# wengflow/robust-e-nerf

Measured on AMD Instinct MI355X. Metric: train_rays_per_sec, higher is better.
Workload: dtype f32; 1 GPU; BASELINE configs[1]: synthetic ficus-like event stream, 65536 events/step/GPU = 2 renders x 65536 rays x 128 samples, arch ngp, fp32, l_diff (2 renders), fwd+bwd+Adam; sampler=uniform; sampler=uniform, samples_per_ray=128, parallelism=dp1, front_prefetched=False, mlp_precision=highest, device_counts=False, device_count_overflows=0, fwd_chunks=8, dist_world_size=1

## Files before the change

robust_e_nerf_amd/csrc/ren_hashgrid_binned.hip:

```cpp
#include <cstdlib>
#include "ren_hashgrid_common.h"

namespace {

constexpr int BIN_SHIFT = 13;
constexpr int BIN_ENTRIES = 1 << BIN_SHIFT;
constexpr int MAX_BINS_PER_LEVEL = 64;
constexpr int MAX_BINS = REN_MAX_LEVELS * MAX_BINS_PER_LEVEL;
#ifndef REN_SC_THREADS
#define REN_SC_THREADS 512
#endif
#ifndef REN_SC_WAVES
#define REN_SC_WAVES 6
#endif
#ifndef REN_SC_WAVES_PAIR
#define REN_SC_WAVES_PAIR 8
#endif
constexpr int SC_THREADS = REN_SC_THREADS;
constexpr int SC_ENTRIES = SC_THREADS * 8;
constexpr int CNT_THREADS = 1024, CNT_SAMPLES = 1024;
constexpr int64_t PART_ENTRIES_MIN = 1 << 16, PART_ENTRIES_MAX = 1 << 23;
constexpr int N_SUB = 8;
__device__ __forceinline__ int xcd_id() {
    unsigned x;
    asm volatile("s_getreg_b32 %0, hwreg(HW_REG_XCC_ID)" : "=s"(x));
    return (int)(x & (N_SUB - 1));
}
inline int64_t part_entries_for(int64_t n, int64_t hashed_cap) {
    int64_t p = hashed_cap;
    if (p == 0) {
        p = PART_ENTRIES_MIN;
        while (p < (1 << 21) && p * 1024 < n * 128) p <<= 1;
    }
    return p < PART_ENTRIES_MIN ? PART_ENTRIES_MIN : (p > PART_ENTRIES_MAX ? PART_ENTRIES_MAX : p);
}
constexpr int LMAX_SLOTS = 8, LMAX_STRIDE = 32;
constexpr int LMAX_WORDS = REN_MAX_LEVELS * LMAX_SLOTS * LMAX_STRIDE;

struct BinTab {
    int bin_base[REN_MAX_LEVELS + 1];
    uint32_t cap[REN_MAX_LEVELS];
    uint32_t pair[REN_MAX_LEVELS];
    uint32_t skip[REN_MAX_LEVELS];
    int sub_by_xcd;
    int cnt_stride;
    int halve;
};

struct Part {
    uint32_t gbin, single;
    uint64_t begin, end;
};

struct Workspace {
    uint32_t *counts, *level_max, *cursors, *n_parts;
    uint32_t *bin_cap;
    uint64_t *bin_start;
    Part *parts;
    char *pool;
};
constexpr int PAIR_BIN_SHIFT = 26;

struct TanSrc {
    const float *rays_do, *rays_dd, *dfeatd;
};

__device__ __forceinline__ void lds_barrier() { asm volatile("s_waitcnt lgkmcnt(0)\n\ts_barrier" ::: "memory"); }

struct SampleArgs {
    int layout;
    const float *dfeat, *x_unit;
    ren_scene_dev sc;
    const float *rays_o, *rays_d;
    const int32_t *ray_indices;
    const float *t_starts, *t_ends;
    int64_t n;
    TanSrc tan;
    const int64_t *n_dev;
};

template <bool TAN>
__device__ __forceinline__ void unit_pos(const SampleArgs &a, int64_t i, float *u, float *ud) {
    ud[0] = 0.f; ud[1] = 0.f; ud[2] = 0.f;
    if (TAN) {
        float x[3], xd[3];
        sample_pos_jvp(a.rays_o, a.rays_d, a.tan.rays_do, a.tan.rays_dd, a.ray_indices, a.t_starts, a.t_ends, i, x, xd);
        contract_jvp(a.sc, x, xd, u, ud);
    } else if (a.x_unit) {
        u[0] = a.x_unit[3 * i]; u[1] = a.x_unit[3 * i + 1]; u[2] = a.x_unit[3 * i + 2];
    } else {
        float x, y, z; int ray;
        ren_sample_pos(a.rays_o, a.rays_d, a.ray_indices, a.t_starts, a.t_ends, i, x, y, z, ray);
        ren_contract(a.sc, x, y, z, u[0], u[1], u[2]);
    }
}

template <bool TAN>
__device__ __forceinline__ bool load_dfeat(const SampleArgs &a, int n_levels, int lvl, int64_t i, float &d0, float &d1,
                                           float &e0, float &e1) {
    e0 = 0.f; e1 = 0.f;
    if (TAN || a.layout == 1) {
        const int64_t b = ((i >> 5) * REN_MAX_LEVELS + lvl) * 64 + (i & 31);
        d0 = a.dfeat[b]; d1 = a.dfeat[b + 32];
        if (TAN) { e0 = a.tan.dfeatd[b]; e1 = a.tan.dfeatd[b + 32]; }
    } else {
        const float2 d = reinterpret_cast<const float2 *>(a.dfeat)[i * n_levels + lvl];
        d0 = d.x; d1 = d.y;
    }
    return d0 != 0.f || d1 != 0.f || e0 != 0.f || e1 != 0.f;
}


constexpr int RUN_LANES = 16;

template <int OFF>
__device__ __forceinline__ float dpp_shr(float v) {
    return __int_as_float(__builtin_amdgcn_update_dpp(0, __float_as_int(v), 0x110 | OFF, 0xf, 0xf, true));
}
template <int OFF>
__device__ __forceinline__ int dpp_shr_i(int v) { return __builtin_amdgcn_update_dpp(0, v, 0x110 | OFF, 0xf, 0xf, true); }

__device__ __forceinline__ bool run_tail(bool dense, bool have, uint32_t key, int lane, bool &head) {
    if (!dense) { head = true; return have; }
    const uint32_t k = have ? key : 0x80000000u | (uint32_t)lane;
    const uint32_t kp = __shfl_up(k, 1, 64), kn = __shfl_down(k, 1, 64);
    const int sub = lane & (RUN_LANES - 1);
    head = !(sub > 0 && have && kp == k);
    return have && (sub == RUN_LANES - 1 || kn != k);
}

template <int OFF>
__device__ __forceinline__ void run_merge_step(int &f, float (&v0)[8], float (&v1)[8]) {
    const float take = f ? 0.f : 1.f;
#pragma unroll
    for (int c = 0; c < 8; ++c) {
        v0[c] = fmaf(dpp_shr<OFF>(v0[c]), take, v0[c]);
        v1[c] = fmaf(dpp_shr<OFF>(v1[c]), take, v1[c]);
    }
    f |= dpp_shr_i<OFF>(f);
}

__device__ __forceinline__ void run_merge(bool head, int lane, float (&v0)[8], float (&v1)[8]) {
    int f = head ? 1 : 0;
    run_merge_step<1>(f, v0, v1);
    run_merge_step<2>(f, v0, v1);
    run_merge_step<4>(f, v0, v1);
    run_merge_step<8>(f, v0, v1);
}

__device__ __forceinline__ uint32_t bin_rank(bool dense, bool emit, uint32_t bin, int lane, uint32_t *hist) {
    if (!dense) return emit ? atomicAdd(&hist[bin], 1u) : 0u;
    uint32_t rank = 0;
    uint64_t todo = __ballot(emit);
    while (todo) {
        const int leader = __ffsll((unsigned long long)todo) - 1;
        const uint32_t b = __shfl(bin, leader, 64);
        const uint64_t m = __ballot(emit && bin == b);
        uint32_t base = 0;
        if (lane == leader) base = atomicAdd(&hist[b], (uint32_t)__popcll(m));
        base = __shfl(base, leader, 64);
        if (emit && bin == b) rank = base + (uint32_t)__popcll(m & ((1ull << lane) - 1ull));
        todo &= ~m;
    }
    return rank;
}

__device__ __forceinline__ void bin_rank8_dense(bool emit, const uint32_t (&bin)[8], int lane, uint32_t *hist, uint32_t (&rank)[8]) {
    const uint64_t m = __ballot(emit);
#pragma unroll
    for (int c = 0; c < 8; ++c) rank[c] = 0;
    if (!m) return;
    const int leader = __ffsll((unsigned long long)m) - 1;
    uint32_t lb[8];
    bool mixed = false;
#pragma unroll
    for (int c = 0; c < 8; ++c) {
        lb[c] = __shfl(bin[c], leader, 64);
        mixed |= emit && bin[c] != lb[c];
    }
    if (__ballot(mixed)) {
#pragma unroll
        for (int c = 0; c < 8; ++c) rank[c] = bin_rank(true, emit, bin[c], lane, hist);
        return;
    }
    const uint32_t cnt = (uint32_t)__popcll(m), pre = (uint32_t)__popcll(m & ((1ull << lane) - 1ull));
    uint32_t base[8] = {0, 0, 0, 0, 0, 0, 0, 0};
    if (lane == leader) {
#pragma unroll
        for (int c = 0; c < 8; ++c) base[c] = atomicAdd(&hist[lb[c]], cnt);
    }
#pragma unroll
    for (int c = 0; c < 8; ++c) rank[c] = __shfl(base[c], leader, 64) + pre;
}

template <bool TAN>
__global__ __launch_bounds__(CNT_THREADS) void bin_count_kernel(GridDev g, BinTab bt, SampleArgs a,
                                                                uint32_t *__restrict__ counts) {
    __shared__ uint32_t hist[MAX_BINS];
    for (int t = threadIdx.x; t < MAX_BINS; t += CNT_THREADS) hist[t] = 0;
    __syncthreads();
    const int lane = threadIdx.x & 63;
#pragma unroll 1
    for (int k = 0; k < CNT_SAMPLES / CNT_THREADS; ++k) {
        const int64_t i = (int64_t)blockIdx.x * bt.cnt_stride * CNT_SAMPLES + k * CNT_THREADS + threadIdx.x;
        const bool inb = i < ren_eff_n(a.n, a.n_dev);
        float u[3] = {0.f, 0.f, 0.f}, ud[3];
        if (inb) unit_pos<TAN>(a, i, u, ud);
#pragma unroll 1
        for (int lvl = 0; lvl < g.n_levels; ++lvl) {
            if (bt.cap[lvl] || bt.skip[lvl]) continue;
            float d0, d1, e0, e1;
            const bool have = inb && (a.dfeat == nullptr || load_dfeat<TAN>(a, g.n_levels, lvl, i, d0, d1, e0, e1));
            const LevelPos p = level_pos(u[0], u[1], u[2], g.scale[lvl]);
            const uint32_t res = g.res[lvl], size = g.size[lvl];
            const bool hashed = g.hashed[lvl] != 0;
            bool head;
            uint32_t idx[8];
            corner_indices8(p.c[0], p.c[1], p.c[2], res, size, hashed, idx);
            const bool emit = run_tail(!hashed, have, idx[0], lane, head);
#pragma unroll
            for (int c = 0; c < 8; ++c) (void)bin_rank(!hashed, emit, idx[c] >> BIN_SHIFT, lane, hist + lvl * MAX_BINS_PER_LEVEL);
        }
    }
    __syncthreads();
    for (int t = threadIdx.x; t < MAX_BINS; t += CNT_THREADS) {
        const int lvl = t / MAX_BINS_PER_LEVEL, bin = t % MAX_BINS_PER_LEVEL;
        if (lvl < g.n_levels && bin < bt.bin_base[lvl + 1] - bt.bin_base[lvl] && hist[t])
            atomicAdd(&counts[bt.bin_base[lvl] + bin], hist[t]);
    }
}

__global__ __launch_bounds__(MAX_BINS) void bin_offsets_kernel(int n_bins, BinTab bt, uint64_t capacity_slots,
                                                               const uint32_t *__restrict__ counts,
                                                               uint32_t *__restrict__ cursors,
                                                               uint32_t *__restrict__ bin_cap,
                                                               uint64_t *__restrict__ bin_start) {
    __shared__ uint64_t s_cnt[MAX_BINS];
    const int t = threadIdx.x;
    uint64_t c = 0, slots = 0;
    bool pair = false;
    if (t < n_bins) {
        int lvl = 0;
        while (lvl + 1 < REN_MAX_LEVELS && t >= bt.bin_base[lvl + 1]) ++lvl;
        pair = bt.pair[lvl] != 0;
        c = bt.skip[lvl] ? 0 : bt.cap[lvl] ? bt.cap[lvl] : counts[t];
        if (!bt.skip[lvl] && !bt.cap[lvl] && bt.cnt_stride > 1) c = c * bt.cnt_stride + c * bt.cnt_stride / 4 + 4096;
        if (bt.halve) c = c / 2;
        c &= ~(uint64_t)7;
        if (pair) c = (c / N_SUB) & ~(uint64_t)7;
        slots = pair ? c * N_SUB : (c * 10 + 15) / 16;
        for (int x = 0; x < N_SUB; ++x) cursors[t * N_SUB + x] = 0;
    }
    s_cnt[t] = slots;
    __syncthreads();
    for (int off = 1; off < MAX_BINS; off <<= 1) {
        const uint64_t a = t >= off ? s_cnt[t - off] : 0;
        __syncthreads();
        s_cnt[t] += a;
        __syncthreads();
    }
    if (t < n_bins) {
        const uint64_t start = s_cnt[t] - slots;
        uint64_t room = start < capacity_slots ? capacity_slots - start : 0;
        if (room > slots) room = slots;
        if (room < slots) c = (pair ? room / N_SUB : room * 16 / 10) & ~(uint64_t)7;
        bin_start[t] = start < capacity_slots ? start : capacity_slots;
        bin_cap[t] = (uint32_t)c;
    }
    if (t == n_bins - 1) bin_start[n_bins] = s_cnt[t] < capacity_slots ? s_cnt[t] : capacity_slots;
}

__global__ __launch_bounds__(MAX_BINS) void bin_partition_kernel(int n_bins, uint64_t PART_ENTRIES, BinTab bt,
                                                                 const uint32_t *__restrict__ cursors,
                                                                 const uint32_t *__restrict__ bin_cap,
                                                                 Part *__restrict__ parts, uint32_t *__restrict__ n_parts) {
    __shared__ uint32_t s_np[MAX_BINS];
    const int t = threadIdx.x;
    uint64_t c = 0;
    bool pair = false;
    if (t < n_bins) {
        int lvl = 0;
        while (lvl + 1 < REN_MAX_LEVELS && t >= bt.bin_base[lvl + 1]) ++lvl;
        pair = bt.pair[lvl] != 0;
        for (int x = 0; x < (pair ? N_SUB : 1); ++x) c += cursors[t * N_SUB + x] < bin_cap[t] ? cursors[t * N_SUB + x] : bin_cap[t];
    }
    const uint32_t np = pair ? (c ? 1u : 0u) : (uint32_t)((c + PART_ENTRIES - 1) / PART_ENTRIES);
    s_np[t] = np;
    __syncthreads();
    for (int off = 1; off < MAX_BINS; off <<= 1) {
        const uint32_t b = t >= off ? s_np[t - off] : 0;
        __syncthreads();
        s_np[t] += b;
        __syncthreads();
    }
    if (t == n_bins - 1) n_parts[0] = s_np[t];
    const uint32_t pbase = s_np[t] - np;
    for (uint32_t k = 0; k < np; ++k) {
        Part p;
        p.gbin = t; p.single = np == 1;
        p.begin = (uint64_t)k * PART_ENTRIES;
        p.end = k + 1 == np ? c : p.begin + PART_ENTRIES;
        parts[pbase + k] = p;
    }
}

__device__ __forceinline__ void table_atomic(float *grad_table, uint32_t offset, uint32_t idx, float a, float b) {
    float *gt = grad_table + 2 * ((size_t)offset + idx);
    atomicAdd(gt, a);
    atomicAdd(gt + 1, b);
}

template <bool TAN, int KIND>
__global__ __launch_bounds__(SC_THREADS, KIND == 1 ? REN_SC_WAVES_PAIR : REN_SC_WAVES) void bin_scatter_kernel(
    GridDev g, BinTab bt, SampleArgs a, Workspace ws, float *__restrict__ grad_table) {
    __shared__ uint32_t hist[MAX_BINS_PER_LEVEL], loc[MAX_BINS_PER_LEVEL + 1], fit[MAX_BINS_PER_LEVEL];
    __shared__ char *gp0[MAX_BINS_PER_LEVEL], *gp1[MAX_BINS_PER_LEVEL];
    __shared__ __attribute__((aligned(16))) unsigned char stage[KIND == 1 ? SC_THREADS * 4 * 16 : SC_ENTRIES * 12];
    __shared__ float wave_max[SC_THREADS / 64];
    __shared__ int any_overflow;
    uint32_t *st_key = reinterpret_cast<uint32_t *>(stage);
    float2 *st_v = reinterpret_cast<float2 *>(stage + SC_ENTRIES * 4);
    float4 *st_p = reinterpret_cast<float4 *>(stage);
    const int64_t chunk = blockIdx.x;
    const int tid = threadIdx.x, lane = tid & 63;
    const int64_t i = chunk * SC_THREADS + tid;
    const bool inb = i < ren_eff_n(a.n, a.n_dev);
    float u[3] = {0.f, 0.f, 0.f}, ud[3] = {0.f, 0.f, 0.f};
    if (inb) unit_pos<TAN>(a, i, u, ud);
    constexpr bool pairs = KIND == 1;
    const int sub = !pairs ? 0 : bt.sub_by_xcd ? xcd_id() : (int)((chunk >> 3) & (N_SUB - 1));
#pragma unroll 1
    for (int lvl = 0; lvl < g.n_levels; ++lvl) {
        if (bt.skip[lvl]) continue;
        if (KIND == 1 && !bt.pair[lvl]) continue;
        if (KIND == 2 && bt.pair[lvl]) continue;
        if (tid < MAX_BINS_PER_LEVEL) hist[tid] = 0;
        if (tid == 0) any_overflow = 0;
        lds_barrier();
        const uint32_t res = g.res[lvl], size = g.size[lvl];
        const bool hashed = g.hashed[lvl] != 0;
        const float scale = g.scale[lvl];
        float d0 = 0.f, d1 = 0.f, e0 = 0.f, e1 = 0.f;
        const bool valid = inb && load_dfeat<TAN>(a, g.n_levels, lvl, i, d0, d1, e0, e1);
        const LevelPos p = level_pos(u[0], u[1], u[2], scale);
        const float wx1 = p.w[0], wy1 = p.w[1], wz1 = p.w[2], wx0 = 1.f - wx1, wy0 = 1.f - wy1, wz0 = 1.f - wz1;
        if (!valid) { d0 = 0.f; d1 = 0.f; e0 = 0.f; e1 = 0.f; }
        uint32_t key[8];
        float v0[8], v1[8];
        bool have;
        float vmax = 0.f;
        uint32_t idx[8];
        corner_indices8(p.c[0], p.c[1], p.c[2], res, size, hashed, idx);
        if (pairs) {
            const bool same = ((idx[0] ^ idx[1]) >> BIN_SHIFT) == 0;
#pragma unroll
            for (int j = 0; j < 4; ++j) {
                const float wyz = ((j & 1) ? wy1 : wy0) * ((j & 2) ? wz1 : wz0);
                v0[j] = wyz * d0; v1[j] = wyz * d1;
            }
            if (valid && !same) {
#pragma unroll
                for (int j = 0; j < 4; ++j) {
                    table_atomic(grad_table, g.offset[lvl], idx[2 * j], wx0 * v0[j], wx0 * v1[j]);
                    table_atomic(grad_table, g.offset[lvl], idx[2 * j + 1], wx1 * v0[j], wx1 * v1[j]);
                }
            }
            have = valid && same;
#pragma unroll
            for (int j = 0; j < 4; ++j) {
                const uint32_t bin = idx[2 * j] >> BIN_SHIFT;
                key[4 + j] = have ? atomicAdd(&hist[bin], 1u) : 0u;
                key[j] = (idx[2 * j] & (BIN_ENTRIES - 1)) | ((idx[2 * j + 1] & (BIN_ENTRIES - 1)) << BIN_SHIFT) |
                         (bin << PAIR_BIN_SHIFT);
            }
            if (valid) vmax = fmaxf(fabsf(d0), fabsf(d1));
        } else {
            const float wxy[4] = {wx0 * wy0, wx1 * wy0, wx0 * wy1, wx1 * wy1};
#pragma unroll
            for (int c = 0; c < 8; ++c) {
                const float wz = (c & 4) ? wz1 : wz0;
                const float w = wxy[c & 3] * wz;
                v0[c] = w * d0; v1[c] = w * d1;
                if (TAN) {
                    const float wx = (c & 1) ? wx1 : wx0, wy = (c & 2) ? wy1 : wy0;
                    const float bx = (c & 1) ? ud[0] : -ud[0], by = (c & 2) ? ud[1] : -ud[1], bz = (c & 4) ? ud[2] : -ud[2];
                    const float wdc = scale * (bx * wy * wz + wx * by * wz + wxy[c & 3] * bz);
                    v0[c] += wdc * e0; v1[c] += wdc * e1;
                }
            }
            bool head;
            have = run_tail(!hashed, valid, idx[0], lane, head);
            if (!hashed) run_merge(head, lane, v0, v1);
            if (TAN) {
                if (have) {
#pragma unroll
                    for (int c = 0; c < 8; ++c) vmax = fmaxf(vmax, fmaxf(fabsf(v0[c]), fabsf(v1[c])));
                }
            } else if (valid) {
                vmax = fmaxf(fabsf(d0), fabsf(d1)) * (hashed ? 1.f : (float)RUN_LANES);
            }
            if (!hashed) {
                uint32_t bins[8], rk[8];
#pragma unroll
                for (int c = 0; c < 8; ++c) bins[c] = idx[c] >> BIN_SHIFT;
                bin_rank8_dense(have, bins, lane, hist, rk);
#pragma unroll
                for (int c = 0; c < 8; ++c) key[c] = (rk[c] << 19) | idx[c];
            } else {
#pragma unroll
                for (int c = 0; c < 8; ++c) {
                    const uint32_t rank = bin_rank(false, have, idx[c] >> BIN_SHIFT, lane, hist);
                    key[c] = (rank << 19) | idx[c];
                }
            }
        }
#pragma unroll
        for (int off = 32; off > 0; off >>= 1) vmax = fmaxf(vmax, __shfl_xor(vmax, off, 64));
        if (lane == 0) wave_max[tid >> 6] = vmax;
        lds_barrier();
        if (tid == SC_THREADS - 1) {
            float m = 0.f;
#pragma unroll
            for (int w = 0; w < SC_THREADS / 64; ++w) m = fmaxf(m, wave_max[w]);
            uint32_t *slot = ws.level_max + (lvl * LMAX_SLOTS + (int)(chunk % LMAX_SLOTS)) * LMAX_STRIDE;
            if (__float_as_uint(m) > __builtin_nontemporal_load(slot)) atomicMax(slot, __float_as_uint(m));
        }
        if (tid < MAX_BINS_PER_LEVEL) {
            const int nb = bt.bin_base[lvl + 1] - bt.bin_base[lvl];
            const uint32_t cnt = hist[tid];
            uint32_t inc = cnt;
#pragma unroll
            for (int off = 1; off < 64; off <<= 1) {
                const uint32_t t = __shfl_up(inc, off, 64);
                if (tid >= off) inc += t;
            }
            loc[tid] = inc - cnt;
            if (tid == MAX_BINS_PER_LEVEL - 1) loc[MAX_BINS_PER_LEVEL] = inc;
            uint32_t room = cnt;
            char *q0 = nullptr, *q1 = nullptr;
            if (tid < nb && cnt) {
                const int gb = bt.bin_base[lvl] + tid;
                const uint32_t at = atomicAdd(&ws.cursors[gb * N_SUB + sub], cnt);
                const uint32_t cap = ws.bin_cap[gb];
                room = at >= cap ? 0u : (cap - at < cnt ? cap - at : cnt);
                char *base = ws.pool + (ws.bin_start[gb] + (pairs ? (uint64_t)sub * cap : 0)) * 16;
                const int64_t first = (int64_t)at - (int64_t)(inc - cnt);
                if (pairs) q0 = base + first * 16;
                else { q0 = base + first * 8; q1 = base + (int64_t)cap * 8 + first * 2; }
            }
            fit[tid] = room;
            if (room < cnt) any_overflow = 1;
            gp0[tid] = q0; gp1[tid] = q1;
        }
        lds_barrier();
        if (have) {
            if (pairs) {
#pragma unroll
                for (int j = 0; j < 4; ++j)
                    st_p[loc[key[j] >> PAIR_BIN_SHIFT] + key[4 + j]] = make_float4(__uint_as_float(key[j]), v0[j], v1[j], wx1);
            } else {
#pragma unroll
                for (int c = 0; c < 8; ++c) {
                    const uint32_t ix = key[c] & 0x7FFFFu;
                    const uint32_t pos = loc[ix >> BIN_SHIFT] + (key[c] >> 19);
                    st_key[pos] = ix;
                    st_v[pos] = make_float2(v0[c], v1[c]);
                }
            }
        }
        lds_barrier();
        const uint32_t total = loc[MAX_BINS_PER_LEVEL];
        const bool ovf = any_overflow != 0;
        if (pairs) {
            for (uint32_t q = tid; q < total; q += SC_THREADS) {
                const float4 r = st_p[q];
                const uint32_t code = __float_as_uint(r.x), b = code >> PAIR_BIN_SHIFT;
                if (!ovf || q - loc[b] < fit[b]) {
                    reinterpret_cast<float4 *>(gp0[b])[q] = r;
                } else {
                    const uint32_t i0 = (b << BIN_SHIFT) | (code & (BIN_ENTRIES - 1));
                    const uint32_t i1 = (b << BIN_SHIFT) | ((code >> BIN_SHIFT) & (BIN_ENTRIES - 1));
                    table_atomic(grad_table, g.offset[lvl], i0, (1.f - r.w) * r.y, (1.f - r.w) * r.z);
                    table_atomic(grad_table, g.offset[lvl], i1, r.w * r.y, r.w * r.z);
                }
            }
            continue;
        }
        for (uint32_t q = tid; q < total; q += SC_THREADS) {
            const uint32_t ix = st_key[q], b = ix >> BIN_SHIFT;
            const float2 v = st_v[q];
            if (!ovf || q - loc[b] < fit[b]) {
                reinterpret_cast<uint16_t *>(gp1[b])[q] = (uint16_t)(ix & (BIN_ENTRIES - 1));
                reinterpret_cast<float2 *>(gp0[b])[q] = v;
            } else {
                table_atomic(grad_table, g.offset[lvl], ix, v.x, v.y);
            }
        }
    }
}

__device__ __forceinline__ long long to_fixed(float v, double scale) {
    return __double2ll_rn((double)v * scale);
}

__global__ __launch_bounds__(1024) void bin_accumulate_kernel(GridDev g, BinTab bt, Workspace ws,
                                                              float *__restrict__ grad_table) {
    extern __shared__ __attribute__((aligned(16))) unsigned long long acc[];
    if (blockIdx.x >= ws.n_parts[0]) return;
    const Part part = ws.parts[blockIdx.x];
    unsigned long long *acc0 = acc, *acc1 = acc + BIN_ENTRIES;
    for (int e = threadIdx.x; e < 2 * BIN_ENTRIES; e += 1024) acc[e] = 0ull;
    int lvl = 0;
    while (lvl + 1 < g.n_levels && (int)part.gbin >= bt.bin_base[lvl + 1]) ++lvl;
    int ex;
    uint32_t lmax = 0;
    for (int k = 0; k < LMAX_SLOTS; ++k) lmax = max(lmax, ws.level_max[(lvl * LMAX_SLOTS + k) * LMAX_STRIDE]);
    (void)frexpf(__uint_as_float(lmax), &ex);
    const double scale = ldexp(1.0, 38 - ex), inv_scale = ldexp(1.0, ex - 38);
    const char *base = ws.pool + ws.bin_start[part.gbin] * 16;
    const uint32_t first = ((uint32_t)part.gbin - bt.bin_base[lvl]) << BIN_SHIFT;
    const uint32_t lim = g.size[lvl] > first ? g.size[lvl] - first : 0;
    float2 *gt = reinterpret_cast<float2 *>(grad_table) + g.offset[lvl] + first;
    constexpr int FL = BIN_ENTRIES / 1024;
    float2 gv[FL];
#pragma unroll
    for (int u = 0; u < FL; ++u) {
        const uint32_t k = threadIdx.x + u * 1024;
        gv[u] = (part.single && k < lim) ? gt[k] : make_float2(0.f, 0.f);
    }
    __syncthreads();
    uint64_t e = part.begin + threadIdx.x;
    if (bt.pair[lvl]) {
        const float4 *rec = reinterpret_cast<const float4 *>(base);
        auto add = [&](const float4 &r) {
            const uint32_t code = __float_as_uint(r.x);
            const uint32_t i0 = code & (BIN_ENTRIES - 1), i1 = (code >> BIN_SHIFT) & (BIN_ENTRIES - 1);
            const float f0 = 1.f - r.w;
            atomicAdd(&acc0[i0], (unsigned long long)to_fixed(f0 * r.y, scale));
            atomicAdd(&acc1[i0], (unsigned long long)to_fixed(f0 * r.z, scale));
            atomicAdd(&acc0[i1], (unsigned long long)to_fixed(r.w * r.y, scale));
            atomicAdd(&acc1[i1], (unsigned long long)to_fixed(r.w * r.z, scale));
        };
        const uint32_t cap = ws.bin_cap[part.gbin];
        for (int x = 0; x < N_SUB; ++x) {
            const float4 *rx = rec + (size_t)x * cap;
            const uint32_t fill = ws.cursors[part.gbin * N_SUB + x];
            const uint64_t end = fill < cap ? fill : cap;
            uint64_t q = threadIdx.x;
            for (; q + 3 * 1024 < end; q += 4 * 1024) {
                float4 r[4];
#pragma unroll
                for (int u = 0; u < 4; ++u) r[u] = rx[q + u * 1024];
#pragma unroll
                for (int u = 0; u < 4; ++u) add(r[u]);
            }
            for (; q < end; q += 1024) add(rx[q]);
        }
    } else {
        const float2 *out_v = reinterpret_cast<const float2 *>(base);
        const uint16_t *out_idx = reinterpret_cast<const uint16_t *>(base + (size_t)ws.bin_cap[part.gbin] * 8);
        for (; e + 3 * 1024 < part.end; e += 4 * 1024) {
            uint32_t ix[4]; float2 v[4];
#pragma unroll
            for (int u = 0; u < 4; ++u) { ix[u] = out_idx[e + u * 1024]; v[u] = out_v[e + u * 1024]; }
#pragma unroll
            for (int u = 0; u < 4; ++u) {
                atomicAdd(&acc0[ix[u]], (unsigned long long)to_fixed(v[u].x, scale));
                atomicAdd(&acc1[ix[u]], (unsigned long long)to_fixed(v[u].y, scale));
            }
        }
        for (; e < part.end; e += 1024) {
            const uint32_t idx = out_idx[e];
            const float2 v = out_v[e];
            atomicAdd(&acc0[idx], (unsigned long long)to_fixed(v.x, scale));
            atomicAdd(&acc1[idx], (unsigned long long)to_fixed(v.y, scale));
        }
    }
    __syncthreads();
#pragma unroll
    for (int u = 0; u < FL; ++u) {
        const uint32_t k = threadIdx.x + u * 1024;
        if (k >= lim) continue;
        const long long qa = (long long)acc0[k], qb = (long long)acc1[k];
        if (qa == 0 && qb == 0) continue;
        const float a = (float)((double)qa * inv_scale), b = (float)((double)qb * inv_scale);
        if (part.single) {
            float2 v = gv[u];
            v.x += a; v.y += b;
            gt[k] = v;
        } else {
            atomicAdd(&gt[k].x, a);
            atomicAdd(&gt[k].y, b);
        }
    }
}

inline size_t align256(size_t v) { return (v + 255) & ~(size_t)255; }

struct Layout { size_t counts, level_max, cursors, n_parts, bin_cap, bin_start, parts, pool, total, slots; int64_t entries, max_parts; };

Layout make_layout(int64_t n) {
    Layout L;
    const size_t E = (size_t)n * 140 + (size_t)MAX_BINS * 4096 + 16 * 8 * 16 * CNT_SAMPLES;
    L.entries = (int64_t)E;
    L.slots = (E * 10 + 15) / 16 + MAX_BINS;
    L.max_parts = (int64_t)(E / PART_ENTRIES_MIN) + MAX_BINS + 1;
    size_t o = 0;
    L.counts = o; o += MAX_BINS * 4;
    L.level_max = o; o = align256(o + LMAX_WORDS * 4);
    L.cursors = o; o = align256(o + MAX_BINS * 4 * N_SUB);
    L.n_parts = o; o = align256(o + 4);
    L.bin_cap = o; o = align256(o + MAX_BINS * 4);
    L.bin_start = o; o = align256(o + (MAX_BINS + 1) * 8);
    L.parts = o; o = align256(o + (size_t)L.max_parts * sizeof(Part));
    L.pool = o; o = align256(o + L.slots * 16);
    L.total = o;
    return L;
}

}

extern "C" int64_t ren_hashgrid_bwd_binned_workspace_bytes(int64_t n) {
    if (n < 0) return -1;
    return (int64_t)make_layout(n).total;
}

static int binned_impl(const ren_grid_desc *grid, float *grad_table, const float *x_unit,
                       const ren_scene_desc *scene, const float *rays_o, const float *rays_d,
                       const int32_t *ray_indices, const float *t_starts, const float *t_ends,
                       int64_t n, int32_t layout, const float *dfeat, void *workspace,
                       void *stream, TanSrc tan, uint32_t level_mask = 0xFFFFFFFFu, int phases = 7,
                       int64_t first = 0, int64_t m = -1, const int64_t *n_dev = nullptr) {
    GridDev g;
    int rc = make_grid(grid, g);
    if (rc) return rc;
    const bool do_begin = phases & 1, do_scatter = phases & 2, do_finish = phases & 4;
    if (m < 0) m = n - first;
    if (!workspace || n < 0 || (layout != 0 && layout != 1) || first < 0 || m < 0 || first + m > n) return REN_ERR_BAD_ARG;
    if ((do_scatter && (!dfeat || !grad_table)) || (do_finish && !grad_table)) return REN_ERR_BAD_ARG;
    if (do_scatter && phases != 7 && ((first & 31) != 0 || tan.dfeatd)) return REN_ERR_BAD_ARG;
    const bool from_rays = x_unit == nullptr;
    if ((do_begin || do_scatter) && from_rays && (!scene || !rays_o || !rays_d || !ray_indices || !t_starts || !t_ends))
        return REN_ERR_BAD_ARG;
    if (layout == 1 && g.n_levels != REN_MAX_LEVELS) return REN_ERR_UNSUPPORTED;
    if (n >= ((int64_t)1 << 28)) return REN_ERR_UNSUPPORTED;
    BinTab bt;
    int nb = 0;
    for (int l = 0; l < REN_MAX_LEVELS; ++l) {
        bt.bin_base[l] = nb;
        if (l < g.n_levels) {
            if (g.size[l] > (uint32_t)(MAX_BINS_PER_LEVEL << BIN_SHIFT)) return REN_ERR_UNSUPPORTED;
            nb += (int)((g.size[l] + BIN_ENTRIES - 1) >> BIN_SHIFT);
        }
    }
    bt.bin_base[REN_MAX_LEVELS] = nb;
    for (int l = g.n_levels; l < REN_MAX_LEVELS; ++l) bt.bin_base[l] = nb;
    int64_t hashed_cap = 0;
    const bool use_pairs = !tan.dfeatd && ren_knob(REN_KNOB_HGB_NO_PAIRS) != 1;
    for (int l = 0; l < REN_MAX_LEVELS; ++l) {
        bt.cap[l] = 0;
        bt.pair[l] = 0;
        bt.skip[l] = l < g.n_levels && !((level_mask >> l) & 1u);
        if (l < g.n_levels && g.hashed[l]) {
            const int64_t bins = (g.size[l] + BIN_ENTRIES - 1) >> BIN_SHIFT;
            bt.pair[l] = use_pairs ? 1 : 0;
            const int64_t mean = ((use_pairs ? 4 : 8) * n + bins - 1) / bins;
            bt.cap[l] = use_pairs ? (uint32_t)(N_SUB * (((mean / N_SUB + mean / 400 + 1024) + 7) & ~(int64_t)7))
                                  : (uint32_t)(mean + mean / 50 + 4096);
            if ((int64_t)bt.cap[l] > hashed_cap) hashed_cap = bt.cap[l];
        }
    }
    const int64_t part_entries = part_entries_for(n, hashed_cap);
    if (n == 0) return REN_OK;
    ren_scene_dev sc = {};
    if (scene) sc = ren_make_scene(scene);
    const Layout L = make_layout(n);
    char *w = (char *)workspace;
    Workspace ws;
    ws.counts = (uint32_t *)(w + L.counts); ws.level_max = (uint32_t *)(w + L.level_max);
    ws.cursors = (uint32_t *)(w + L.cursors);
    ws.n_parts = (uint32_t *)(w + L.n_parts); ws.bin_cap = (uint32_t *)(w + L.bin_cap);
    ws.bin_start = (uint64_t *)(w + L.bin_start);
    ws.parts = (Part *)(w + L.parts); ws.pool = w + L.pool;
    hipStream_t st = (hipStream_t)stream;
    SampleArgs a;
    a.layout = layout; a.dfeat = dfeat; a.x_unit = x_unit; a.sc = sc; a.rays_o = rays_o; a.rays_d = rays_d;
    a.ray_indices = ray_indices; a.t_starts = t_starts; a.t_ends = t_ends; a.n = n; a.tan = tan;
    a.n_dev = n_dev;
    if (n_dev && phases != 7) return REN_ERR_BAD_ARG;
    bt.halve = ren_knob(REN_KNOB_HGB_HALVE_REGIONS) == 1;
    bt.sub_by_xcd = ren_knob(REN_KNOB_HGB_SUBREGION) != 0;
    const int64_t cnt_blocks = (n + CNT_SAMPLES - 1) / CNT_SAMPLES;
    bt.cnt_stride = cnt_blocks >= 4096 ? 16 : cnt_blocks >= 2048 ? 8 : cnt_blocks >= 1024 ? 4 : 1;
    bool any_pair = false, any_single = false;
    for (int l = 0; l < g.n_levels; ++l)
        if (!bt.skip[l]) { any_pair |= bt.pair[l] != 0; any_single |= bt.pair[l] == 0; }
    if (do_begin) {
        if (hipMemsetAsync(ws.counts, 0, (MAX_BINS + LMAX_WORDS) * 4, st) != hipSuccess) return REN_ERR_LAUNCH;
        const dim3 cgrd((unsigned)((cnt_blocks + bt.cnt_stride - 1) / bt.cnt_stride)), cblk(CNT_THREADS);
        SampleArgs ac = a;
        if (phases != 7) ac.dfeat = nullptr;
        if (tan.dfeatd) hipLaunchKernelGGL(bin_count_kernel<true>, cgrd, cblk, 0, st, g, bt, ac, ws.counts);
        else            hipLaunchKernelGGL(bin_count_kernel<false>, cgrd, cblk, 0, st, g, bt, ac, ws.counts);
        hipLaunchKernelGGL(bin_offsets_kernel, dim3(1), dim3(MAX_BINS), 0, st, nb, bt, (uint64_t)L.slots, ws.counts,
                           ws.cursors, ws.bin_cap, ws.bin_start);
    }
    if (!any_pair && !any_single) return REN_OK;
    if (do_scatter && m > 0) {
        SampleArgs as = a;
        as.n = m;
        if (first) {
            if (as.x_unit) as.x_unit += 3 * first;
            if (as.ray_indices) { as.ray_indices += first; as.t_starts += first; as.t_ends += first; }
            as.dfeat += layout == 1 ? (first >> 5) * (int64_t)(REN_MAX_LEVELS * 64) : first * (int64_t)g.n_levels * 2;
        }
        const dim3 sgrd((unsigned)((m + SC_THREADS - 1) / SC_THREADS)), sblk(SC_THREADS);
        if (tan.dfeatd) hipLaunchKernelGGL((bin_scatter_kernel<true, 0>), sgrd, sblk, 0, st, g, bt, as, ws, grad_table);
        else {
            if (any_pair)   hipLaunchKernelGGL((bin_scatter_kernel<false, 1>), sgrd, sblk, 0, st, g, bt, as, ws, grad_table);
            if (any_single) hipLaunchKernelGGL((bin_scatter_kernel<false, 2>), sgrd, sblk, 0, st, g, bt, as, ws, grad_table);
        }
    }
    if (do_finish) {
        hipLaunchKernelGGL(bin_partition_kernel, dim3(1), dim3(MAX_BINS), 0, st, nb, (uint64_t)part_entries, bt, ws.cursors, ws.bin_cap, ws.parts,
                           ws.n_parts);
        const size_t acc_lds = 2 * BIN_ENTRIES * sizeof(unsigned long long);
        (void)hipFuncSetAttribute((const void *)bin_accumulate_kernel, hipFuncAttributeMaxDynamicSharedMemorySize, (int)acc_lds);
        const int64_t acc_grid = (int64_t)(L.entries / part_entries) + nb + 1;
        hipLaunchKernelGGL(bin_accumulate_kernel, dim3((unsigned)acc_grid), dim3(1024), acc_lds, st, g, bt, ws, grad_table);
    }
    REN_CHECK_LAUNCH();
}

extern "C" int ren_hashgrid_bwd_binned(const ren_grid_desc *grid, float *grad_table, const float *x_unit,
                                       const ren_scene_desc *scene, const float *rays_o, const float *rays_d,
                                       const int32_t *ray_indices, const float *t_starts, const float *t_ends,
                                       int64_t n, int32_t layout, const float *dfeat, void *workspace,
                                       const int64_t *n_dev, void *stream) {
    return binned_impl(grid, grad_table, x_unit, scene, rays_o, rays_d, ray_indices, t_starts, t_ends, n, layout,
                       dfeat, workspace, stream, TanSrc{nullptr, nullptr, nullptr}, 0xFFFFFFFFu, 7, 0, -1, n_dev);
}

extern "C" int ren_hashgrid_bwd_binned_jvp(const ren_grid_desc *grid, float *grad_table,
                                           const ren_scene_desc *scene, const float *rays_o, const float *rays_d,
                                           const float *rays_do, const float *rays_dd, const int32_t *ray_indices,
                                           const float *t_starts, const float *t_ends, int64_t n,
                                           const float *dfeat, const float *dfeatd, void *workspace, void *stream) {
    if (!rays_do || !rays_dd || !dfeatd) return REN_ERR_BAD_ARG;
    return binned_impl(grid, grad_table, nullptr, scene, rays_o, rays_d, ray_indices, t_starts, t_ends, n, 1, dfeat,
                       workspace, stream, TanSrc{rays_do, rays_dd, dfeatd});
}

extern "C" int ren_hashgrid_bwd_binned_levels(const ren_grid_desc *grid, float *grad_table, const float *x_unit,
                                              const ren_scene_desc *scene, const float *rays_o, const float *rays_d,
                                              const int32_t *ray_indices, const float *t_starts, const float *t_ends,
                                              int64_t n, int32_t layout, const float *dfeat, const float *rays_do,
                                              const float *rays_dd, const float *dfeatd, uint32_t level_mask,
                                              void *workspace, const int64_t *n_dev, void *stream) {
    if ((rays_do || rays_dd || dfeatd) && (!rays_do || !rays_dd || !dfeatd || layout != 1 || x_unit)) return REN_ERR_BAD_ARG;
    return binned_impl(grid, grad_table, x_unit, scene, rays_o, rays_d, ray_indices, t_starts, t_ends, n, layout, dfeat,
                       workspace, stream, TanSrc{rays_do, rays_dd, dfeatd}, level_mask, 7, 0, -1, n_dev);
}

extern "C" int ren_hashgrid_bwd_binned_begin(const ren_grid_desc *grid, const float *x_unit, const ren_scene_desc *scene,
                                             const float *rays_o, const float *rays_d, const int32_t *ray_indices,
                                             const float *t_starts, const float *t_ends, int64_t n, int32_t layout,
                                             void *workspace, void *stream) {
    return binned_impl(grid, nullptr, x_unit, scene, rays_o, rays_d, ray_indices, t_starts, t_ends, n, layout, nullptr,
                       workspace, stream, TanSrc{nullptr, nullptr, nullptr}, 0xFFFFFFFFu, 1);
}

extern "C" int ren_hashgrid_bwd_binned_scatter(const ren_grid_desc *grid, float *grad_table, const float *x_unit,
                                               const ren_scene_desc *scene, const float *rays_o, const float *rays_d,
                                               const int32_t *ray_indices, const float *t_starts, const float *t_ends,
                                               int64_t n, int32_t layout, const float *dfeat, int64_t first, int64_t m,
                                               void *workspace, void *stream) {
    return binned_impl(grid, grad_table, x_unit, scene, rays_o, rays_d, ray_indices, t_starts, t_ends, n, layout, dfeat,
                       workspace, stream, TanSrc{nullptr, nullptr, nullptr}, 0xFFFFFFFFu, 2, first, m);
}

extern "C" int ren_hashgrid_bwd_binned_finish(const ren_grid_desc *grid, float *grad_table, int64_t n, int32_t layout,
                                              void *workspace, void *stream) {
    return binned_impl(grid, grad_table, nullptr, nullptr, nullptr, nullptr, nullptr, nullptr, nullptr, n, layout, nullptr,
                       workspace, stream, TanSrc{nullptr, nullptr, nullptr}, 0xFFFFFFFFu, 4);
}
```

Measured before the change: 6.123 million rays/s.

## Rank whole dense cells with one LDS atomic per bin and DPP run detection

For dense (non-hashed) single levels, the scatter kernel now checks whether all 8 corners of a sample's cell fall in one bin and form the expected contiguous span. Such 'whole' cells reserve 8 contiguous staging slots with a single per-bin LDS atomic per wave, instead of ranking each corner separately. Other cells still use per-corner ranking. Run-tail detection switches to DPP row shifts in place of cross-lane shuffles. The old path stays reachable through a knob value; the new path adds ballot loops and a branch that may cost more when few cells are whole.

```diff
diff --git a/robust_e_nerf_amd/csrc/ren_hashgrid_binned.hip b/robust_e_nerf_amd/csrc/ren_hashgrid_binned.hip
--- a/robust_e_nerf_amd/csrc/ren_hashgrid_binned.hip
+++ b/robust_e_nerf_amd/csrc/ren_hashgrid_binned.hip
@@ -191,6 +191,42 @@
     }
 #pragma unroll
     for (int c = 0; c < 8; ++c) rank[c] = __shfl(base[c], leader, 64) + pre;
+}
+
+
+template <int CTRL>
+__device__ __forceinline__ uint32_t dpp_u(uint32_t v) {
+    return (uint32_t)__builtin_amdgcn_update_dpp(0, (int)v, CTRL, 0xf, 0xf, true);
+}
+
+__device__ __forceinline__ bool run_tail_row(bool have, uint32_t key, int lane, bool &head) {
+    const uint32_t k = have ? key : 0x80000000u | (uint32_t)lane;
+    const uint32_t kp = dpp_u<0x111>(k), kn = dpp_u<0x101>(k);
+    const int sub = lane & (RUN_LANES - 1);
+    head = !(sub > 0 && have && kp == k);
+    return have && (sub == RUN_LANES - 1 || kn != k);
+}
+
+__device__ __forceinline__ uint32_t cell_rank(bool emit, bool whole, const uint32_t (&idx)[8], int lane, uint32_t *hist,
+                                              uint32_t (&rank)[8]) {
+    const uint32_t bin = idx[0] >> BIN_SHIFT;
+    uint32_t first = 0;
+    uint64_t todo = __ballot(emit && whole);
+    while (todo) {
+        const int leader = __ffsll((unsigned long long)todo) - 1;
+        const uint32_t b = (uint32_t)__builtin_amdgcn_readlane((int)bin, leader);
+        const uint64_t m = todo & __ballot(bin == b);
+        uint32_t base = 0;
+        if (lane == leader) base = atomicAdd(&hist[b], 8u * (uint32_t)__popcll(m));
+        base = (uint32_t)__builtin_amdgcn_readlane((int)base, leader);
+        if ((m >> lane) & 1) first = base + 8u * (uint32_t)__popcll(m & ((1ull << lane) - 1ull));
+        todo &= ~m;
+    }
+    if (__ballot(emit && !whole)) {
+#pragma unroll
+        for (int c = 0; c < 8; ++c) rank[c] = bin_rank(true, emit && !whole, idx[c] >> BIN_SHIFT, lane, hist);
+    }
+    return first;
 }
 
 template <bool TAN>
@@ -327,13 +363,13 @@
     const bool inb = i < ren_eff_n(a.n, a.n_dev);
     float u[3] = {0.f, 0.f, 0.f}, ud[3] = {0.f, 0.f, 0.f};
     if (inb) unit_pos<TAN>(a, i, u, ud);
-    constexpr bool pairs = KIND == 1;
+    constexpr bool pairs = KIND == 1, cells = KIND == 2;
     const int sub = !pairs ? 0 : bt.sub_by_xcd ? xcd_id() : (int)((chunk >> 3) & (N_SUB - 1));
 #pragma unroll 1
     for (int lvl = 0; lvl < g.n_levels; ++lvl) {
         if (bt.skip[lvl]) continue;
         if (KIND == 1 && !bt.pair[lvl]) continue;
-        if (KIND == 2 && bt.pair[lvl]) continue;
+        if (KIND >= 2 && bt.pair[lvl]) continue;
         if (tid < MAX_BINS_PER_LEVEL) hist[tid] = 0;
         if (tid == 0) any_overflow = 0;
         lds_barrier();
@@ -347,7 +383,8 @@
         if (!valid) { d0 = 0.f; d1 = 0.f; e0 = 0.f; e1 = 0.f; }
         uint32_t key[8];
         float v0[8], v1[8];
-        bool have;
+        bool have, whole = false;
+        uint32_t first = 0;
         float vmax = 0.f;
         uint32_t idx[8];
         corner_indices8(p.c[0], p.c[1], p.c[2], res, size, hashed, idx);
@@ -389,7 +426,8 @@
                 }
             }
             bool head;
-            have = run_tail(!hashed, valid, idx[0], lane, head);
+            if (cells && !hashed) have = run_tail_row(valid, idx[0], lane, head);
+            else have = run_tail(!hashed, valid, idx[0], lane, head);
             if (!hashed) run_merge(head, lane, v0, v1);
             if (TAN) {
                 if (have) {
@@ -399,7 +437,14 @@
             } else if (valid) {
                 vmax = fmaxf(fabsf(d0), fabsf(d1)) * (hashed ? 1.f : (float)RUN_LANES);
             }
-            if (!hashed) {
+            if (cells && !hashed) {
+                const uint32_t span = dense_stride_y(res, size) + dense_stride_z(res, size) + 1u;
+                whole = idx[7] - idx[0] == span && ((idx[0] ^ idx[7]) >> BIN_SHIFT) == 0;
+                uint32_t rk[8] = {0, 0, 0, 0, 0, 0, 0, 0};
+                first = cell_rank(have, whole, idx, lane, hist, rk);
+#pragma unroll
+                for (int c = 0; c < 8; ++c) key[c] = (rk[c] << 19) | idx[c];
+            } else if (!hashed) {
                 uint32_t bins[8], rk[8];
 #pragma unroll
                 for (int c = 0; c < 8; ++c) bins[c] = idx[c] >> BIN_SHIFT;
@@ -458,6 +503,13 @@
 #pragma unroll
                 for (int j = 0; j < 4; ++j)
                     st_p[loc[key[j] >> PAIR_BIN_SHIFT] + key[4 + j]] = make_float4(__uint_as_float(key[j]), v0[j], v1[j], wx1);
+            } else if (cells && whole) {
+                const uint32_t pos = loc[key[0] >> BIN_SHIFT] + first;
+#pragma unroll
+                for (int c = 0; c < 8; ++c) {
+                    st_key[pos + c] = key[c];
+                    st_v[pos + c] = make_float2(v0[c], v1[c]);
+                }
             } else {
 #pragma unroll
                 for (int c = 0; c < 8; ++c) {
@@ -718,7 +770,10 @@
         if (tan.dfeatd) hipLaunchKernelGGL((bin_scatter_kernel<true, 0>), sgrd, sblk, 0, st, g, bt, as, ws, grad_table);
         else {
             if (any_pair)   hipLaunchKernelGGL((bin_scatter_kernel<false, 1>), sgrd, sblk, 0, st, g, bt, as, ws, grad_table);
-            if (any_single) hipLaunchKernelGGL((bin_scatter_kernel<false, 2>), sgrd, sblk, 0, st, g, bt, as, ws, grad_table);
+            if (any_single && ren_knob(REN_KNOB_HGB_NO_PAIRS) == 2)
+                hipLaunchKernelGGL((bin_scatter_kernel<false, 3>), sgrd, sblk, 0, st, g, bt, as, ws, grad_table);
+            else if (any_single)
+                hipLaunchKernelGGL((bin_scatter_kernel<false, 2>), sgrd, sblk, 0, st, g, bt, as, ws, grad_table);
         }
     }
     if (do_finish) {
```

New measurement: 6.176 million rays/s, median of 2. No clear change (+0.9%).

## Add lean path for non-tangent single-corner binned scatter with DPP reductions and fewer barriers

Applied to the files above, without the earlier changes.

For the non-paired, non-tangent scatter kernel, this adds a lean path. It clears the bin histogram once up front and resets it during the scan, which removes one barrier per level. It also prefetches the next level's feature gradients, and swaps shuffle-based merges, scans and max reductions for DPP inline-asm fmac, readlane and row-shift sequences. Validity is now inferred from a nonzero gradient rather than from load_dfeat's return value. That could change behaviour if a valid sample has an exactly zero gradient, and the hand-written DPP asm with s_nop hazards is fragile.

```diff
diff --git a/robust_e_nerf_amd/csrc/ren_hashgrid_binned.hip b/robust_e_nerf_amd/csrc/ren_hashgrid_binned.hip
--- a/robust_e_nerf_amd/csrc/ren_hashgrid_binned.hip
+++ b/robust_e_nerf_amd/csrc/ren_hashgrid_binned.hip
@@ -191,6 +191,80 @@
     }
 #pragma unroll
     for (int c = 0; c < 8; ++c) rank[c] = __shfl(base[c], leader, 64) + pre;
+}
+
+
+#define REN_FMAC_SHR(OFF)                                                                                              \
+    "s_nop 4\n\t"                                                                                                      \
+    "v_fmac_f32_dpp %0, %0, %8 row_shr:" #OFF " row_mask:0xf bank_mask:0xf bound_ctrl:1\n\t"                             \
+    "v_fmac_f32_dpp %1, %1, %8 row_shr:" #OFF " row_mask:0xf bank_mask:0xf bound_ctrl:1\n\t"                             \
+    "v_fmac_f32_dpp %2, %2, %8 row_shr:" #OFF " row_mask:0xf bank_mask:0xf bound_ctrl:1\n\t"                             \
+    "v_fmac_f32_dpp %3, %3, %8 row_shr:" #OFF " row_mask:0xf bank_mask:0xf bound_ctrl:1\n\t"                             \
+    "v_fmac_f32_dpp %4, %4, %8 row_shr:" #OFF " row_mask:0xf bank_mask:0xf bound_ctrl:1\n\t"                             \
+    "v_fmac_f32_dpp %5, %5, %8 row_shr:" #OFF " row_mask:0xf bank_mask:0xf bound_ctrl:1\n\t"                             \
+    "v_fmac_f32_dpp %6, %6, %8 row_shr:" #OFF " row_mask:0xf bank_mask:0xf bound_ctrl:1\n\t"                             \
+    "v_fmac_f32_dpp %7, %7, %8 row_shr:" #OFF " row_mask:0xf bank_mask:0xf bound_ctrl:1"
+#define REN_FMAC_SHR8(OFF, v)                                                                                          \
+    asm(REN_FMAC_SHR(OFF)                                                                                              \
+        : "+v"(v[0]), "+v"(v[1]), "+v"(v[2]), "+v"(v[3]), "+v"(v[4]), "+v"(v[5]), "+v"(v[6]), "+v"(v[7])               \
+        : "v"(take))
+
+__device__ __forceinline__ void run_merge_fmac(bool head, float (&v0)[8], float (&v1)[8]) {
+    int f = head ? 1 : 0;
+    float take = f ? 0.f : 1.f;
+    REN_FMAC_SHR8(1, v0); REN_FMAC_SHR8(1, v1);
+    f |= dpp_shr_i<1>(f); take = f ? 0.f : 1.f;
+    REN_FMAC_SHR8(2, v0); REN_FMAC_SHR8(2, v1);
+    f |= dpp_shr_i<2>(f); take = f ? 0.f : 1.f;
+    REN_FMAC_SHR8(4, v0); REN_FMAC_SHR8(4, v1);
+    f |= dpp_shr_i<4>(f); take = f ? 0.f : 1.f;
+    REN_FMAC_SHR8(8, v0); REN_FMAC_SHR8(8, v1);
+}
+
+__device__ __forceinline__ uint32_t lane_value(uint32_t v, int uniform_lane) {
+    return (uint32_t)__builtin_amdgcn_readlane((int)v, uniform_lane);
+}
+
+__device__ __forceinline__ void bin_rank8_dense_rl(bool emit, const uint32_t (&bin)[8], int lane, uint32_t *hist, uint32_t (&rank)[8]) {
+    const uint64_t m = __ballot(emit);
+#pragma unroll
+    for (int c = 0; c < 8; ++c) rank[c] = 0;
+    if (!m) return;
+    const int leader = __ffsll((unsigned long long)m) - 1;
+    uint32_t lb[8];
+    bool mixed = false;
+#pragma unroll
+    for (int c = 0; c < 8; ++c) {
+        lb[c] = lane_value(bin[c], leader);
+        mixed |= emit && bin[c] != lb[c];
+    }
+    if (__ballot(mixed)) {
+#pragma unroll
+        for (int c = 0; c < 8; ++c) rank[c] = bin_rank(true, emit, bin[c], lane, hist);
+        return;
+    }
+    const uint32_t cnt = (uint32_t)__popcll(m), pre = (uint32_t)__popcll(m & ((1ull << lane) - 1ull));
+    uint32_t base[8] = {0, 0, 0, 0, 0, 0, 0, 0};
+    if (lane == leader) {
+#pragma unroll
+        for (int c = 0; c < 8; ++c) base[c] = atomicAdd(&hist[bin[c]], cnt);
+    }
+#pragma unroll
+    for (int c = 0; c < 8; ++c) rank[c] = lane_value(base[c], leader) + pre;
+}
+
+__device__ __forceinline__ uint32_t wave_scan_incl(uint32_t x, int lane) {
+    int v = (int)x;
+    v += dpp_shr_i<1>(v); v += dpp_shr_i<2>(v); v += dpp_shr_i<4>(v); v += dpp_shr_i<8>(v);
+    const uint32_t t0 = lane_value((uint32_t)v, 15), t1 = lane_value((uint32_t)v, 31), t2 = lane_value((uint32_t)v, 47);
+    return (uint32_t)v + (lane >= 16 ? t0 : 0u) + (lane >= 32 ? t1 : 0u) + (lane >= 48 ? t2 : 0u);
+}
+
+__device__ __forceinline__ float wave_max_nonneg(float x) {
+    x = fmaxf(x, dpp_shr<1>(x)); x = fmaxf(x, dpp_shr<2>(x)); x = fmaxf(x, dpp_shr<4>(x)); x = fmaxf(x, dpp_shr<8>(x));
+    const uint32_t b = __float_as_uint(x);
+    return fmaxf(fmaxf(__uint_as_float(lane_value(b, 15)), __uint_as_float(lane_value(b, 31))),
+                 fmaxf(__uint_as_float(lane_value(b, 47)), __uint_as_float(lane_value(b, 63))));
 }
 
 template <bool TAN>
@@ -329,19 +403,40 @@
     if (inb) unit_pos<TAN>(a, i, u, ud);
     constexpr bool pairs = KIND == 1;
     const int sub = !pairs ? 0 : bt.sub_by_xcd ? xcd_id() : (int)((chunk >> 3) & (N_SUB - 1));
+    constexpr bool lean = KIND == 2 && !TAN;
+    if (lean) {
+        if (tid < MAX_BINS_PER_LEVEL) hist[tid] = 0;
+        lds_barrier();
+    }
+    float pd0 = 0.f, pd1 = 0.f;
+    int pl = -1;
 #pragma unroll 1
     for (int lvl = 0; lvl < g.n_levels; ++lvl) {
         if (bt.skip[lvl]) continue;
         if (KIND == 1 && !bt.pair[lvl]) continue;
         if (KIND == 2 && bt.pair[lvl]) continue;
-        if (tid < MAX_BINS_PER_LEVEL) hist[tid] = 0;
-        if (tid == 0) any_overflow = 0;
-        lds_barrier();
+        if (!lean) {
+            if (tid < MAX_BINS_PER_LEVEL) hist[tid] = 0;
+            if (tid == 0) any_overflow = 0;
+            lds_barrier();
+        }
         const uint32_t res = g.res[lvl], size = g.size[lvl];
         const bool hashed = g.hashed[lvl] != 0;
         const float scale = g.scale[lvl];
         float d0 = 0.f, d1 = 0.f, e0 = 0.f, e1 = 0.f;
-        const bool valid = inb && load_dfeat<TAN>(a, g.n_levels, lvl, i, d0, d1, e0, e1);
+        bool valid;
+        if (lean) {
+            float t0, t1;
+            if (pl != lvl && inb) (void)load_dfeat<TAN>(a, g.n_levels, lvl, i, pd0, pd1, t0, t1);
+            d0 = pd0; d1 = pd1;
+            int nl = lvl + 1;
+            while (nl < g.n_levels && (bt.skip[nl] || bt.pair[nl])) ++nl;
+            pl = nl;
+            if (nl < g.n_levels && inb) (void)load_dfeat<TAN>(a, g.n_levels, nl, i, pd0, pd1, t0, t1);
+            valid = inb && (d0 != 0.f || d1 != 0.f);
+        } else {
+            valid = inb && load_dfeat<TAN>(a, g.n_levels, lvl, i, d0, d1, e0, e1);
+        }
         const LevelPos p = level_pos(u[0], u[1], u[2], scale);
         const float wx1 = p.w[0], wy1 = p.w[1], wz1 = p.w[2], wx0 = 1.f - wx1, wy0 = 1.f - wy1, wz0 = 1.f - wz1;
         if (!valid) { d0 = 0.f; d1 = 0.f; e0 = 0.f; e1 = 0.f; }
@@ -390,7 +485,10 @@
             }
             bool head;
             have = run_tail(!hashed, valid, idx[0], lane, head);
-            if (!hashed) run_merge(head, lane, v0, v1);
+            if (!hashed) {
+                if (lean) run_merge_fmac(head, v0, v1);
+                else run_merge(head, lane, v0, v1);
+            }
             if (TAN) {
                 if (have) {
 #pragma unroll
@@ -403,7 +501,8 @@
                 uint32_t bins[8], rk[8];
 #pragma unroll
                 for (int c = 0; c < 8; ++c) bins[c] = idx[c] >> BIN_SHIFT;
-                bin_rank8_dense(have, bins, lane, hist, rk);
+                if (lean) bin_rank8_dense_rl(have, bins, lane, hist, rk);
+                else bin_rank8_dense(have, bins, lane, hist, rk);
 #pragma unroll
                 for (int c = 0; c < 8; ++c) key[c] = (rk[c] << 19) | idx[c];
             } else {
@@ -414,8 +513,12 @@
                 }
             }
         }
-#pragma unroll
-        for (int off = 32; off > 0; off >>= 1) vmax = fmaxf(vmax, __shfl_xor(vmax, off, 64));
+        if (lean) {
+            vmax = wave_max_nonneg(vmax);
+        } else {
+#pragma unroll
+            for (int off = 32; off > 0; off >>= 1) vmax = fmaxf(vmax, __shfl_xor(vmax, off, 64));
+        }
         if (lane == 0) wave_max[tid >> 6] = vmax;
         lds_barrier();
         if (tid == SC_THREADS - 1) {
@@ -429,10 +532,15 @@
             const int nb = bt.bin_base[lvl + 1] - bt.bin_base[lvl];
             const uint32_t cnt = hist[tid];
             uint32_t inc = cnt;
-#pragma unroll
-            for (int off = 1; off < 64; off <<= 1) {
-                const uint32_t t = __shfl_up(inc, off, 64);
-                if (tid >= off) inc += t;
+            if (lean) {
+                hist[tid] = 0;
+                inc = wave_scan_incl(cnt, lane);
+            } else {
+#pragma unroll
+                for (int off = 1; off < 64; off <<= 1) {
+                    const uint32_t t = __shfl_up(inc, off, 64);
+                    if (tid >= off) inc += t;
+                }
             }
             loc[tid] = inc - cnt;
             if (tid == MAX_BINS_PER_LEVEL - 1) loc[MAX_BINS_PER_LEVEL] = inc;
@@ -449,7 +557,10 @@
                 else { q0 = base + first * 8; q1 = base + (int64_t)cap * 8 + first * 2; }
             }
             fit[tid] = room;
-            if (room < cnt) any_overflow = 1;
+            if (lean) {
+                const bool o = __ballot(room < cnt) != 0;
+                if (tid == 0) any_overflow = o ? 1 : 0;
+            } else if (room < cnt) any_overflow = 1;
             gp0[tid] = q0; gp1[tid] = q1;
         }
         lds_barrier();
```

Result: no change. 6.175 million rays/s before, 6.228 million rays/s after (median of 6 runs) (+0.9%).
